# mateog4712/CCJ

Hardware: AMD Instinct MI355X
Metric: sec/sequence + DP-cells/s at n=200 (Turner04), 1/2/4/8 GPU vs CPU ref (higher is better)
Workload: dtype int32

## Files before the change

### ccj_amd/__init__.py

```python
from __future__ import annotations

import ctypes
import os
from typing import Optional

__all__ = [
    "W_final", "ccj", "load_params", "load_par", "ParFileError", "param_path", "CCJError", "BacktrackExit", "lib", "MAT4", "MAT2",
    "num_cells", "comm_unique_id", "shard_blocks", "level_layout", "level_schedule", "LevelSchedule",
    "DEFAULT_SPLIT_TARGET", "LocalGroup", "W_final_pf", "PF_MAT4", "PF_MAT2", "layout_extents", "fold_many",
    "SampleExit", "pf_exp_hashes", "load_pfraw", "LockstepBatch", "batch_level_plan", "BatchLevelPlan", "plan_lockstep",
    "pf_many", "PfLockstepBatch", "pf_level_plan", "PF_PLAN_KERNELS", "pf_setup_host_hashes", "PF_SETUP_TABLES", "RangeError", "RANGE_LEVEL", "RANGE_ILOOP", "RANGE_PARTIAL", "RANGE_TAB", "RANGE_CF", "RANGE_EXIT_CODE",
]

_HERE = os.path.dirname(os.path.abspath(__file__))
_VARIANT = os.environ.get("CCJ_LIB_VARIANT", "")
_LIB_PATH = os.path.join(_HERE, "lib", f"libccj_hip_{_VARIANT}.so" if _VARIANT else "libccj_hip.so")
PARAM_DIR = os.path.join(_HERE, "params")

MAT4 = ["PK", "PL", "PR", "PM", "PO", "PfromL", "PfromR", "PfromM", "PfromMprime", "PfromO",
        "PLmloop00", "PLmloop01", "PLmloop10", "PRmloop00", "PRmloop01", "PRmloop10",
        "PMmloop00", "PMmloop01", "PMmloop10", "POmloop00", "POmloop01", "POmloop10"]
MAT2 = ["P", "WBP", "WPP", "V", "Vtype", "WM", "WMv", "WMp"]
HASH_NAMES = MAT4 + MAT2 + ["W"]
PF_MAT4 = ["PK", "PL", "PR", "PM", "PO", "PfromL", "PfromR", "PfromM", "PfromO",
           "PLmloop00", "PLmloop01", "PLmloop10", "PRmloop00", "PRmloop01", "PRmloop10",
           "PMmloop00", "PMmloop01", "PMmloop10", "POmloop00", "POmloop01", "POmloop10"]
PF_MAT2 = ["V", "VM", "WM", "WMv", "WMp", "WBP", "WPP", "P"]
CCJ_E_PF_SAMPLE = 8
CCJ_E_PF_RANGE = 10

CCJ_OK, CCJ_E_ARG, CCJ_E_OOM, CCJ_E_HIP, CCJ_E_PARAMS, CCJ_E_BACKTRACK, CCJ_E_STATE, CCJ_E_INTER_EXIT = range(8)
CCJ_E_COMM = 9
CCJ_E_PARFILE = 8
CCJ_E_RANGE = 11
RANGE_LEVEL, RANGE_ILOOP, RANGE_PARTIAL, RANGE_TAB, RANGE_CF = 1, 2, 4, 8, 16
RANGE_SITES = {"LEVEL": RANGE_LEVEL, "ILOOP": RANGE_ILOOP, "PARTIAL": RANGE_PARTIAL, "TAB": RANGE_TAB, "CF": RANGE_CF}
RANGE_EXIT_CODE = 3

PARAM_SETS = {
    "Turner04": "Turner04.ccjp", "rna_Turner04": "Turner04.ccjp",
    "DirksPierce09": "DirksPierce09.ccjp", "rna_DirksPierce09": "DirksPierce09.ccjp",
    "DirksPierce03": "DirksPierce03.ccjp", "rna_DirksPierce03": "DirksPierce03.ccjp",
    "CaoChen06": "CaoChen06.ccjp", "rna_CaoChen06": "CaoChen06.ccjp",
    "CaoChen09": "CaoChen09.ccjp", "rna_CaoChen09": "CaoChen09.ccjp",
# ... 171 lines not shown
        L.ccj_pf_reset.restype = ip
        L.ccj_pf_capacity.argtypes = [vp]
        L.ccj_pf_capacity.restype = ip
        L.ccj_pf_n.argtypes = [vp]
        L.ccj_pf_n.restype = ip
        L.ccj_pf_keytab_info.argtypes = [vp, dp, ctypes.POINTER(ctypes.c_ulonglong)]
        L.ccj_pf_keytab_info.restype = ip
        L.ccj_pf_setup_hashes.argtypes = [vp, u64p, ip]
        L.ccj_pf_setup_hashes.restype = ip
        L.ccj_pf_setup_host_hashes.argtypes = [ctypes.POINTER(_Problem), cp, u64p, u64p]
        L.ccj_pf_setup_host_hashes.restype = ip
    if hasattr(L, "ccj_pf_batch_create"):
        L.ccj_pf_batch_create.argtypes = [ctypes.POINTER(_Problem), cp, ip, ip, ip, ctypes.POINTER(vp)]
        L.ccj_pf_batch_create.restype = ip
        L.ccj_pf_batch_bind.argtypes = [vp, ctypes.POINTER(cp), ip]
        L.ccj_pf_batch_bind.restype = ip
        for fn in ("ccj_pf_batch_fill", "ccj_pf_batch_members", "ccj_pf_batch_count", "ccj_pf_batch_launches"):
            getattr(L, fn).argtypes = [vp]
            getattr(L, fn).restype = ip
        L.ccj_pf_batch_result.argtypes = [vp, ip, dp]
        L.ccj_pf_batch_result.restype = ip
        L.ccj_pf_batch_member.argtypes = [vp, ip]
        L.ccj_pf_batch_member.restype = vp
        L.ccj_pf_batch_fill_ms.argtypes = [vp]
        L.ccj_pf_batch_fill_ms.restype = ctypes.c_double
        L.ccj_pf_batch_item_counts.argtypes = [vp, ip, ctypes.POINTER(ip)]
        L.ccj_pf_batch_item_counts.restype = ip
        L.ccj_pf_batch_last_error.argtypes = [vp]
        L.ccj_pf_batch_last_error.restype = cp
        L.ccj_pf_batch_destroy.argtypes = [vp]
        L.ccj_pf_batch_destroy.restype = None
        L.ccj_pf_level_plan_items.argtypes = [ctypes.POINTER(ip), ctypes.POINTER(ip), ip, ip, ctypes.POINTER(ip)]
        L.ccj_pf_level_plan_items.restype = ip
    L.ccj_pf_fill.argtypes = [vp, dp]
    L.ccj_pf_fill.restype = ip
    L.ccj_pf_W.argtypes = [vp, dp]
    L.ccj_pf_W.restype = ip
    L.ccj_pf_get2.argtypes = [vp, ip, dp]
    L.ccj_pf_get2.restype = ip
    L.ccj_pf_get4.argtypes = [vp, ip, ip, ip, ip, ip, ctypes.POINTER(ip)]
    L.ccj_pf_get4.restype = ip
    L.ccj_pf_hashes.argtypes = [vp, u64p, u64p]
    L.ccj_pf_hashes.restype = ip
    L.ccj_pf_exp_hashes.argtypes = [vp, u64p, ip]
    L.ccj_pf_exp_hashes.restype = ip
    L.ccj_pf_exp_hashes_params.argtypes = [cp, cp, vp, u64p, ip]
    L.ccj_pf_exp_hashes_params.restype = ip
    L.ccj_pf_exp_names.argtypes = []
    L.ccj_pf_exp_names.restype = cp
    L.ccj_pf_srand.argtypes = [vp, ctypes.c_uint]
    L.ccj_pf_srand.restype = ip
    L.ccj_pf_sample.argtypes = [vp, ip, cp, ctypes.POINTER(ip)]
    L.ccj_pf_sample.restype = ip
    L.ccj_pf_last_message.argtypes = [vp]
    L.ccj_pf_last_message.restype = cp
    L.ccj_pf_timing.argtypes = [vp, ctypes.POINTER(ctypes.c_float)]
    L.ccj_pf_timing.restype = ip
    L.ccj_pf_set_timing.argtypes = [vp, ip]
    L.ccj_pf_set_timing.restype = ip
    L.ccj_pf_kernel_ms.argtypes = [vp, ctypes.POINTER(ctypes.c_double)]
    L.ccj_pf_kernel_ms.restype = ip
    L.ccj_pf_work_model.argtypes = [vp, ctypes.POINTER(ctypes.c_double)]
    L.ccj_pf_work_model.restype = ip
    _lib = L
    return L


def num_cells(n: int) -> int:
    if n < 3:
        return 0
    m = n + 1
    return m * (m - 1) * (m - 2) * (m - 3) // 24


def param_path(name_or_path: str) -> str:
    if os.path.exists(name_or_path) and name_or_path.endswith(".ccjp"):
        return name_or_path
    base = os.path.basename(name_or_path)
    for suf in (".par", ".ccjp"):
        if base.endswith(suf):
            base = base[: -len(suf)]
    if base in PARAM_SETS:
        return os.path.join(PARAM_DIR, PARAM_SETS[base])
    raise CCJError(CCJ_E_ARG, f"unknown parameter set {name_or_path!r}")


class ParFileError(CCJError):

    def __init__(self, log: str):
        super().__init__(CCJ_E_PARFILE, log)
        self.log = log


def load_par(path: str, base: bytes | None = None, text: bool = False):
    if base is None:
        base = _read_blob(os.path.join(PARAM_DIR, "default.ccjp"))
    L = lib()
    out = ctypes.create_string_buffer(len(base))
    cap = 1 << 22
    log = ctypes.create_string_buffer(cap)
    fn = L.ccj_params_load_par_string if text else L.ccj_params_load_par
    rc = fn(path.encode(), bytes(base), out, log, cap)
    msg = log.value.decode(errors="replace")
    if rc == CCJ_E_PARFILE:
        raise ParFileError(msg)
# ... 66 lines not shown

    def reset(self, seq: str) -> None:
        if len(seq) != self.n:
            raise CCJError(CCJ_E_ARG, f"reset: length {len(seq)} differs from n={self.n}")
        self._check(lib().ccj_reset(self._h, seq.encode()))
        self.seq = seq
        self._seq_buf = ctypes.create_string_buffer(seq.encode())
        self.structure = None
        self.energy = None
        self.stdout_msgs = ""

    def rebind(self, seq: str) -> None:
        self._check(lib().ccj_rebind(self._h, seq.encode()))
        self.seq = seq
        self.n = len(seq)
        self._seq_buf = ctypes.create_string_buffer(seq.encode())
        self.structure = None
        self.energy = None
        self.stdout_msgs = ""

    @property
    def capacity(self) -> int:
        return lib().ccj_capacity(self._h)

    def _check(self, rc: int):
        if rc == CCJ_E_RANGE:
            raise RangeError(rc, lib().ccj_last_error(self._h).decode(), self.range_flags())
        if rc != CCJ_OK:
            raise CCJError(rc, lib().ccj_last_error(self._h).decode())

    def range_flags(self) -> int:
        return lib().ccj_range_flags(self._h)

    def fill(self):
        self._check(lib().ccj_fill(self._h))

    def fill_device(self):
        self._check(lib().ccj_fill_device(self._h))

    def sync_host(self):
        self._check(lib().ccj_sync_host(self._h))

    def result(self):
        L = lib()
        buf = ctypes.create_string_buffer(self.n + 1)
        msgs = ctypes.create_string_buffer(1 << 16)
        e = ctypes.c_double()
        rc = L.ccj_result(self._h, buf, ctypes.byref(e), msgs, 1 << 16)
        self.stdout_msgs = msgs.value.decode()
        if rc == CCJ_E_BACKTRACK or rc == CCJ_E_INTER_EXIT:
            err = L.ccj_last_error(self._h).decode()
            exit_code = 0 if rc == CCJ_E_INTER_EXIT else (134 if "Assertion" in err else 1)
            raise BacktrackExit(rc, err, exit_code, self.stdout_msgs)
        self._check(rc)
        self.structure = buf.value.decode()
        self.energy = e.value
        return self.energy

    def ccj(self) -> float:
        self.fill()
        return self.result()

    def fill_async(self, after: Optional["W_final"] = None) -> None:
        if after is None:
            self._check(lib().ccj_fill_async(self._h))
        else:
# ... 692 lines not shown
```

### ccj_amd/csrc/ccj_host.cc

```cpp
#include <hip/hip_runtime.h>
#include <rccl/rccl.h>

#include <algorithm>
#include <atomic>
#include <chrono>
#include <condition_variable>
#include <mutex>
#include <cmath>
#include <cstdarg>
#include <cstdio>
#include <cstdlib>
#include <cstring>
#include <list>
#include <memory>
#include <stack>
#include <string>
#include <thread>
#include <vector>

#include "ccj.h"
#include "ccj_energy.h"
#include "ccj_engine.h"
#include "ccj_backtrack.h"
#include "ccj_traceback.h"
#include "ccj_items.h"

using namespace ccj;

namespace {

const int BP_PAIR[8][8] = {{0, 0, 0, 0, 0, 0, 0, 0}, {0, 0, 0, 0, 5, 0, 0, 5}, {0, 0, 0, 1, 0, 0, 0, 0},
                           {0, 0, 2, 0, 3, 0, 0, 0}, {0, 6, 0, 4, 0, 0, 0, 6}, {0, 0, 0, 0, 0, 0, 2, 0},
                           {0, 0, 0, 0, 0, 1, 0, 0}, {0, 6, 0, 0, 5, 0, 0, 0}};

template <class T>
struct DevBuf {
    T *p = nullptr;
    size_t count = 0;
};

}

struct ccj_group {
    int world = 1;
    std::vector<ccj_ctx *> members;
    std::mutex mu;
    std::condition_variable cv;
    int arrived = 0;
    long gen = 0;
    bool broken = false;
    int busy = 0;
    int range_acc[2] = {0, 0};
    bool barrier() {
        std::unique_lock<std::mutex> lk(mu);
        if (broken) return false;
        const long g = gen;
        if (++arrived == world) {
            arrived = 0;
// ... 1890 lines not shown

extern "C" int ccj_work_model(const ccj_ctx *c, double *out) {
    if (!c || !out) return CCJ_E_ARG;
    double w[5];
    const int rc = work_model(c->n, c->S.data(), c->pair, w);
    for (int x = 0; x < 4; ++x) out[x] = w[x];
    return rc;
}

extern "C" int ccj_work_split(const ccj_ctx *c, double *out2) {
    if (!c || !out2) return CCJ_E_ARG;
    double w[5];
    const int rc = work_model(c->n, c->S.data(), c->pair, w);
    out2[0] = 2.0 * w[4];
    out2[1] = w[0] - out2[0];
    return rc;
}

extern "C" int ccj_work_model_seq(const char *seq, int noGU, double *out) {
    if (!seq || !out) return CCJ_E_ARG;
    const int n = (int)strlen(seq);
    int pairt[8][8];
    for (int x = 0; x < 8; ++x)
        for (int y = 0; y < 8; ++y) pairt[x][y] = BP_PAIR[x][y];
    if (noGU) pairt[3][4] = pairt[4][3] = 0;
    std::vector<short> S(n + 2, 0);
    for (int i = 1; i <= n; ++i) S[i] = (short)encode_base(seq[i - 1]);
    double w[5];
    const int rc = work_model(n, S.data(), pairt, w);
    for (int x = 0; x < 4; ++x) out[x] = w[x];
    return rc;
}

extern "C" int ccj_host_timing(const ccj_ctx *c, double *out3) {
    if (!c || !out3) return CCJ_E_ARG;
    out3[0] = c->sync_ms;
    out3[1] = c->w_ms;
    out3[2] = c->bt_ms;
    return CCJ_OK;
}

extern "C" int ccj_level_times(const ccj_ctx *c, double *level_ms, double *diag_ms, int cap) {
    if (!c) return CCJ_E_ARG;
    for (int t = 0; t < cap && t < (int)c->lev_ms_v.size(); ++t) {
        if (level_ms) level_ms[t] = c->lev_ms_v[t];
        if (diag_ms) diag_ms[t] = c->diag_ms_v[t];
    }
    return CCJ_OK;
}

extern "C" int ccj_iloop_times(const ccj_ctx *c, double *iloop_ms, int cap) {
    if (!c || !iloop_ms) return CCJ_E_ARG;
    for (int t = 0; t < cap && t < (int)c->il_ms_v.size(); ++t) iloop_ms[t] = c->il_ms_v[t];
    return CCJ_OK;
}

extern "C" int ccj_exchange_times(const ccj_ctx *c, double *edge_ms, double *bulk_ms, int cap) {
    if (!c || (!edge_ms && !bulk_ms)) return CCJ_E_ARG;
    for (int t = 0; t < cap && t < (int)c->xch_ms_v.size(); ++t) {
        if (edge_ms) edge_ms[t] = c->xch_ms_v[t];
        if (bulk_ms) bulk_ms[t] = c->xbulk_ms_v[t];
    }
    return CCJ_OK;
}

extern "C" double ccj_iloop_ms(const ccj_ctx *c) { return c ? c->il_ms : 0.0; }
// ... 499 lines not shown
```

### ccj_amd/csrc/ccj_kernels.hip

```cpp
#include <hip/hip_runtime.h>
#include <stdlib.h>
#include "ccj_engine.h"
#include "ccj_energy.h"
#include "ccj_items.h"

using namespace ccj;

#ifdef CCJ_WG_TIMELINE
constexpr int TL_CAP = 1 << 15, TL_KINDS = 8;
__device__ int g_tl_level = -1;
__device__ ulonglong4 g_tl[TL_KINDS][TL_CAP];
struct TLStamp {
    int slot;
    unsigned long long t0;
    unsigned meta = 0xffffffffu;
    template <class K>
    __device__ __forceinline__ explicit TLStamp(K kind_of) {
        const int kind = kind_of(g_tl_level);
        const int wpb = (int)(blockDim.x >> 6);
        const int s = (int)blockIdx.x * wpb + (int)(threadIdx.x >> 6);
        slot = (g_tl_level >= 0 && kind >= 0 && s < TL_CAP && (threadIdx.x & 63) == 0) ? kind * TL_CAP + s : -1;
        t0 = __builtin_amdgcn_s_memrealtime();
    }
    __device__ __forceinline__ ~TLStamp() {
        if (slot < 0) return;
        const unsigned long long t1 = __builtin_amdgcn_s_memrealtime();
        const unsigned hw = __builtin_amdgcn_s_getreg((31 << 11) | 4);
        (&g_tl[0][0])[slot] = make_ulonglong4(t0, t1, meta, hw | (unsigned long long)(blockIdx.x % 8) << 32);
    }
};
#define TL_STAMP(expr_) TLStamp tl_stamp_([&](int L_) -> int { return (expr_); })
#define TL_META(v_) (tl_stamp_.meta = (unsigned)(v_))
#else
#define TL_STAMP(expr_)
#define TL_META(v_)
#endif

// ... 109 lines not shown
            if (e != INF) e += E_MLstem(P, tt, -1, -1) + P->MLclosing;
            break;
    }
    return e;
}

}

__device__ __forceinline__ void init2d_body(const DevTables &T, int total) {
    for (int x = blockIdx.x * blockDim.x + threadIdx.x; x < total; x += gridDim.x * blockDim.x) {
        T.V[x] = 10000;
        T.Vt[x] = 'N';
        T.WM[x] = T.WMv[x] = T.WMp[x] = INF + 1;
        T.P[x] = T.WBP[x] = T.WPP[x] = INF + 1;
        T.Pk[x] = ~0ull;
        T.WB[x] = 0;
        T.WP[x] = 0;
        T.WBW[x] = make_int2(INF + 1, 0);
#pragma unroll
        for (int f = 0; f < 6; ++f) T.tab[f * T.tabN + x] = (int16_t)INTERN_INF;
#pragma unroll
        for (int f = 0; f < NCF; ++f) T.cf[f * T.tabN + x] = INF;
    }
}
__global__ void k_init2d(DevTables T, int total) { init2d_body(T, total); }
__global__ void k_init2d_many(const DevTables *__restrict__ tabs) {
    const DevTables &T = tabs[blockIdx.y];
    init2d_body(T, (T.n + 1) * T.rs);
}

__device__ __forceinline__ int e_intP(const DevTables &T, int u1, int u2, int p, int q) {
    const int d = p + u1 + 1, dp = q - u2 - 1;
    if (dp - d < 1) return INTERN_INF;
    const int t1 = T.pair[T.S[p] * 8 + T.S[q]];
    const int t2 = T.pair[T.S[d] * 8 + T.S[dp]];
    if (t1 <= 0 || t2 <= 0) return INTERN_INF;
    const int e = E_IntLoop(T.prm, T.lx, u1, u2, t1, T.rtype[t2], T.S1[p + 1], T.S1[q - 1], T.S1[d - 1], T.S1[dp + 1]);
    const int v = (int)rint(T.e_intP * (double)e);
    if (v < -32768 || v >= INTERN_INF) atomicOr(T.err, 1);
    return v;
}

__device__ __forceinline__ void precompute_ie_body(const DevTables &T) {
    const int n = T.n, rs = T.rs;
    const int w = blockIdx.y;
    for (int p = 1 + blockIdx.x * blockDim.x + threadIdx.x; p + w <= n; p += gridDim.x * blockDim.x)
        T.ie[(size_t)w * rs + p] = (int16_t)e_intP(T, 0, 0, p, p + w);
}
__global__ void k_precompute_ie(DevTables T) { precompute_ie_body(T); }
__global__ void k_precompute_ie_many(const DevTables *__restrict__ tabs) { precompute_ie_body(tabs[blockIdx.z]); }

__device__ __forceinline__ void diag2d_tables(const DevTables &T, int sigma, int item) {
    const int n = T.n, rs = T.rs, w = sigma;
    const int p = 1 + item, q = p + w;
    if (q > n) return;
    const int lane = threadIdx.x & 63;
    const int cp = T.pen.cp;
    const int16_t *F00 = T.tab, *F10 = T.tab + 2 * T.tabN, *G00 = T.tab + 3 * T.tabN;
    Mloop2dAcc L = mloop2d_begin(T.pen.bp), R = L;
    for (int s = 1 + lane; s <= w; s += 64) {
#ifdef CCJ_DEBUG_BOUNDS
        if (p + s > n || q - s + 1 < 1 || w - s < 0) atomicOr(T.err, 512);
#endif
        const int head = T.WBW[(s - 1) * rs + p].x, tail = T.WBW[(s - 1) * rs + q - s + 1].x;
        const int o = (w - s) * rs + p;
        mloop2d_step(L, true, s, w, cp, head, tail, F00[o + s], F00[o], F10[o]);
        mloop2d_step(R, false, s, w, cp, head, tail, G00[o + s], G00[o], 0);
    }
    L.m00 = wave_min(L.m00); L.m01 = wave_min(L.m01); L.m10 = wave_min(L.m10);
    R.m00 = wave_min(R.m00); R.m01 = wave_min(R.m01); R.m10 = wave_min(R.m10);
    if (lane != 0) return;
    if (w >= 1) {
// ... 414 lines not shown
                for (int s = 0; s < PP_S; ++s) {
                    const int code = (live && s < ns && hh[u] <= o0 + s) ? 1023 - hh[u] : PP_OFF;
                    bv[s] = imin(bv[s], ((va[u][s] + vb[u]) << 10) + code);
                }
            }
        }
#pragma unroll
        for (int s = 0; s < PP_S; ++s) {
            const int sg = lev + 3 + o0 + s;
            const int i = l - sg;
            if (s < ns && l <= n && i >= 1 && bv[s] < (PP_OFF >> 1)) {
                const unsigned h2 = 1023u - (unsigned)(bv[s] & 1023);
                const unsigned jo = (unsigned)(o0 + s) - h2, dd = jo + 1u + (unsigned)a2, ko = dd + 1u + h2;
                const unsigned key = (jo * (unsigned)sg + dd) * (unsigned)sg + ko;
                atomicMin(T.Pk + sg * rs + i, ((unsigned long long)((unsigned)(bv[s] >> 10) + 0x80000000u) << 32) | key);
            }
        }
    }
}
constexpr int PPUSH_HS = 32;
template <int PP_S, int PP_U>
__global__ __launch_bounds__(256) void k_ppush(DevTables T, int lev, int ngrp, int npairs, int hs_len, int blocksA, int G,
                                               int rank, int nout) {
    ppush_body<PP_S, PP_U>(T, lev, ngrp, npairs, hs_len, blocksA, G, rank, nout);
}
template <int PP_S, int PP_U>
__global__ __launch_bounds__(256) void k_ppush_many(const DevTables *__restrict__ tabs, const LevelArgs *__restrict__ args,
                                                    int lev) {
    const LevelArgs &A = args[blockIdx.y];
    if ((int)blockIdx.x >= 2 * A.pp_blocksA) return;
    ppush_body<PP_S, PP_U>(tabs[blockIdx.y], lev, A.pp_ngrp, A.pp_npairs, PPUSH_HS, A.pp_blocksA, 1, 0, A.pp_nout);
}

__device__ __forceinline__ void build_il_body(const DevTables &T, int kind) {
    __shared__ int16_t es[IE_U][IE_U + 1];
    __shared__ uint32_t vb[IE_U];
    const int n = T.n, rs = T.rs;
    const int p = blockIdx.x + 1, w = blockIdx.y;
    const int q = p + w;
    if (q > n) return;
    if (T.pt[(size_t)w * rs + p] <= 0) return;
    const int lane = threadIdx.x;
    const size_t pidx = (size_t)w * rs + p;
    uint32_t *seg = (kind ? T.ilmseg : T.ilseg) + pidx * IL_SEG;
    uint2 *ent = (kind ? T.ilm : T.il) + pidx * IL_CAP;
    if (lane < IE_U) {
        const int u1 = lane;
        uint32_t bits = 0;
#pragma unroll
        for (int u2 = 0; u2 < IE_U; ++u2) {
            bool valid = false;
            int e = 0;
            if (kind == 0) {
                const int d = p + 1 + u1, dp = q - 1 - u2;
                if (u1 <= imin(w, MAXLOOP) - 2 && u2 <= imin(w - u1 - 6, MAXLOOP - 2) && T.pt[(dp - d) * rs + d] > 0) {
                    valid = true;
                    e = e_intP(T, u1, u2, p, q);
                }
            } else {
                const int d = p - 1 - u1, dp = q + 1 + u2;
                if (d >= 1 && dp <= n && T.pt[(dp - d) * rs + d] > 0) {
                    valid = true;
                    e = e_intP(T, u1, u2, d, dp);
                }
            }
            es[u1][u2] = (int16_t)e;
            bits |= (valid ? 1u : 0u) << u2;
        }
        vb[u1] = bits;
    }
    __syncthreads();
    int cnt = 0;
    for (int dt = 0; dt < IL_SEG; ++dt) {
        if (lane == 0) seg[dt] = (uint32_t)cnt;
        const int u1 = lane, u2 = dt - 2 - lane;
        const bool valid = dt >= 2 && u1 < IE_U && u2 >= 0 && u2 < IE_U && ((vb[u1] >> u2) & 1u);
        const unsigned long long mask = __ballot(valid);
        if (valid)
            ent[cnt + __popcll(mask & ((1ull << lane) - 1))] =
                make_uint2(((uint32_t)dt << 21) | ((uint32_t)u1 << 16) | (uint32_t)(uint16_t)es[u1][u2], (uint32_t)(2 * u1 * dt));
        cnt += __popcll(mask);
    }
    if (lane < IL_B) ent[cnt + lane] = make_uint2((63u << 21) | (uint32_t)INTERN_INF, 0u);
}
__global__ __launch_bounds__(64) void k_build_il(DevTables T) { build_il_body(T, (int)blockIdx.z); }
__global__ __launch_bounds__(64) void k_build_il_many(const DevTables *__restrict__ tabs) {
    build_il_body(tabs[blockIdx.z >> 1], (int)(blockIdx.z & 1));
}

struct DevPT {
    const DevTables *T;
    __device__ int operator()(int i, int j) const { return ptype(*T, i, j); }
};

__global__ __launch_bounds__(256) void k_items(DevTables T, int G, int rank, int simulate,
                                               long long *counts, const long long *__restrict__ offs, uint32_t *items,
                                               int pass) {
    __shared__ int wsum[4];
    __shared__ long long tot;
    const int bs = blockIdx.x, b = bs / KI_SPLIT, sp = bs - b * KI_SPLIT, t = b / G, r = b - t * G;
    const int tid = threadIdx.x, lane = tid & 63, w = tid >> 6;
    const bool mine = simulate || r == rank;
    if (!mine || t < 4 || t >= T.nlev) {
        if (pass == 0 && tid == 0) counts[bs] = 0;
        return;
    }
    const ItemRows R = item_rows(T.n, t, G, r);
    const DevPT pt{&T};
    int lo, hi;
    ki_split_rows(R.nPL + R.nPR + R.nPM, sp, lo, hi);
    long long base = pass ? offs[bs] : 0;
    for (int c0 = lo; c0 < hi; c0 += 256) {
        const int x = c0 + tid;
        uint32_t it0 = 0;
        const int cnt = x < hi ? item_row(pt, T.n, t, R, x, G, r, it0, IL_CW) : 0;
        int inc = cnt;
#pragma unroll
        for (int o = 1; o < 64; o <<= 1) {
            const int y = __shfl_up(inc, o, 64);
            if (lane >= o) inc += y;
// ... 1088 lines not shown
}

static bool ppush_geom(int n, int lev, int G, int rank, int &ngrp, int &npairs, int &nout, int &blocksA) {
    ngrp = npairs = nout = blocksA = 0;
    const int nmax = imin(lev, n - 4 - lev) + 1;
    if (nmax <= 0) return false;
    ngrp = (n - lev - 3 + 63) / 64;
    constexpr int S = PPUSH_S, hs_len = PPUSH_HS;
    const int nch = (nmax + S - 1) / S;
    for (int c = 0; c < nch; ++c) npairs += (imin((c + 1) * S, nmax) + hs_len - 1) / hs_len;
    nout = rank <= lev ? (lev - rank) / G + 1 : 0;
    if (nout <= 0) return false;
    blocksA = (npairs * ngrp * nout + 3) / 4;
    return true;
}

extern "C" int ccjk_ppush(const DevTables *T, int lev, int G, int rank, void *stream) {
#ifdef CCJ_ABLATE_PTERM
    return 0;
#endif
    constexpr int S = PPUSH_S, hs_len = PPUSH_HS;
    int ngrp, npairs, nout, blocksA;
    if (!ppush_geom(T->n, lev, G, rank, ngrp, npairs, nout, blocksA)) return 0;
    static const int steps = getenv("CCJ_PP_STEPS") ? atoi(getenv("CCJ_PP_STEPS")) : 4;
    if (steps >= 4)
        hipLaunchKernelGGL((k_ppush<S, 4>), dim3((unsigned)(2 * blocksA)), dim3(256), 0, (hipStream_t)stream, *T, lev, ngrp,
                           npairs, hs_len, blocksA, G, rank, nout);
    else
        hipLaunchKernelGGL((k_ppush<S, 2>), dim3((unsigned)(2 * blocksA)), dim3(256), 0, (hipStream_t)stream, *T, lev, ngrp,
                           npairs, hs_len, blocksA, G, rank, nout);
    return (int)hipGetLastError();
}

extern "C" int ccjk_build_il(const DevTables *T, void *stream) {
    const int n = T->n;
    if (n < 1) return 0;
    hipLaunchKernelGGL(k_build_il, dim3(n, n + 1, 2), dim3(64), 0, (hipStream_t)stream, *T);
    return (int)hipGetLastError();
}

extern "C" int ccjk_iloop(const DevTables *T, int t, long long first_item, int nitems, int G, int rank, void *stream) {
#ifdef CCJ_ABLATE_ILOOP
    return 0;
#endif
    if (nitems <= 0) return 0;
    hipLaunchKernelGGL(k_iloop, dim3((unsigned)((nitems + IL_WPB - 1) / IL_WPB)), dim3(64 * IL_WPB), 0, (hipStream_t)stream, *T, t, first_item,
                       nitems, G, rank);
    return (int)hipGetLastError();
}

__global__ __launch_bounds__(256) void k_pack(DevTables T, int t, int G, int r, int part, int nmax, int16_t *send) {
    const int n = T.n, m = n - t - 2, Mt = (m * (m + 1)) >> 1;
    const long long gc = (long long)blockIdx.x * blockDim.x + threadIdx.x;
    const int k = (int)(gc / Mt);
    if (k >= xch_pcount(t, G, r, part)) return;
    const int c = (int)(gc - (long long)k * Mt);
    const LvlDev Lt = T.ld[t];
    const int16_t *src = T.d4 + Lt.lb + (long long)shard_a(xch_own(k, part), G, r) * Mt + c;
#pragma unroll 2
    for (int x = 0; x < NMAT4; ++x) {
        const bool own = carrier(x) == IN_D4 || carrier(x) == IN_REC;
        send[xch_pos(x, k, c, nmax, Mt)] = own ? src[(long long)mslot(x) * Lt.C] : (int16_t)INTERN_INF;
    }
}

__global__ __launch_bounds__(256) void k_unpack(DevTables T, int t, int G, int r, int part, int nmax, const int16_t *recv,
                                                size_t rstride) {
    const int n = T.n, m = n - t - 2, Mt = (m * (m + 1)) >> 1;
    const long long gc = (long long)blockIdx.x * blockDim.x + threadIdx.x;
    const int a = (int)(gc / Mt);
// ... 259 lines not shown
    for (int k = 0; k < count; ++k) {
        const int m = n[k] - t - 2;
        if (m > 0) total += (long)(t + 1) * ((m * (m + 1) / 2 + 63) / 64);
    }
    BatchLevelPlan P{0, 0, 0, 0};
    if (total <= 0 || t < 0) {
        for (int k = 0; k < count; ++k) {
            if (blocks) blocks[k] = 0;
            if (wpa) wpa[k] = 0;
        }
        return P;
    }
    P.split = sched_split_of(total, split_target);
    P.threads = P.split <= 4 ? 256 : 64 * P.split;
    const int cpb = P.threads / 64 / P.split;
    P.lds = P.split > 1 ? cpb * (P.split - 1) * SPLIT_RED * 64 * (int)sizeof(int) : 0;
    for (int k = 0; k < count; ++k) {
        const int m = n[k] - t - 2;
        const int w = m > 0 ? (m * (m + 1) / 2 + 63) / 64 : 0;
        const long b = ((long)(m > 0 ? t + 1 : 0) * w + cpb - 1) / cpb;
        if (blocks) blocks[k] = (int)b;
        if (wpa) wpa[k] = w;
        P.gridx = b > P.gridx ? (int)b : P.gridx;
    }
    return P;
}

extern "C" int ccjk_pre_many(const DevTables *tabs, int count, int nmax, void *stream) {
    if (count <= 0 || nmax < 1) return 0;
    const hipStream_t s = (hipStream_t)stream;
    const int total = (nmax + 1) * (nmax + 2);
    hipLaunchKernelGGL(k_init2d_many, dim3((total + 255) / 256, count), dim3(256), 0, s, tabs);
    hipLaunchKernelGGL(k_precompute_ie_many, dim3((nmax + 255) / 256, nmax + 1, count), dim3(256), 0, s, tabs);
    hipLaunchKernelGGL(k_build_il_many, dim3(nmax, nmax + 1, 2 * count), dim3(64), 0, s, tabs);
    return (int)hipGetLastError();
}

extern "C" int ccjk_iloop_many(const DevTables *tabs, const LevelArgs *row, const LevelArgs *hrow, int count, int t, void *stream) {
    int gx = 0;
    for (int k = 0; k < count; ++k) gx = imax(gx, (hrow[k].il_nitems + IL_WPB - 1) / IL_WPB);
    if (gx <= 0) return 0;
    hipLaunchKernelGGL(k_iloop_many, dim3(gx, count), dim3(64 * IL_WPB), 0, (hipStream_t)stream, tabs, row, t);
    return (int)hipGetLastError();
}

extern "C" int ccjk_diag2d_many(const DevTables *tabs, const LevelArgs *row, const LevelArgs *hrow, int count, int sigma,
                                void *stream) {
    int gx = 0;
    for (int k = 0; k < count; ++k) gx = imax(gx, hrow[k].dg_blocks);
    if (gx <= 0) return 0;
    hipLaunchKernelGGL(k_diag2d_many, dim3(gx, count), dim3(256), 0, (hipStream_t)stream, tabs, row, sigma);
    return (int)hipGetLastError();
}

extern "C" int ccjk_level4d_many(const DevTables *tabs, const LevelArgs *row, const int *n, int count, int t, int split_target,
                                 void *stream) {
    const BatchLevelPlan P = ccjk_batch_level_plan(n, count, t, split_target, nullptr, nullptr);
    if (P.gridx <= 0) return 0;
    hipLaunchKernelGGL(k_level4d_many, dim3((unsigned)P.gridx, count), dim3(P.threads), (size_t)P.lds, (hipStream_t)stream, tabs,
                       row, t, P.split);
    return (int)hipGetLastError();
}

extern "C" int ccjk_ppush_many(const DevTables *tabs, const LevelArgs *row, const LevelArgs *hrow, int count, int lev,
                               void *stream) {
#ifdef CCJ_ABLATE_PTERM
    return 0;
// ... 23 lines not shown
```

### include/ccj.h

```cpp
#ifndef CCJ_H
#define CCJ_H

#include <stdint.h>
#include "ccj_params.h"

#ifdef __cplusplus
extern "C" {
#endif

#define CCJ_OK           0
#define CCJ_E_ARG        1
#define CCJ_E_OOM        2
#define CCJ_E_HIP        3
#define CCJ_E_PARAMS     4
#define CCJ_E_BACKTRACK  5
#define CCJ_E_STATE      6
#define CCJ_E_INTER_EXIT 7
#define CCJ_E_COMM       9
#define CCJ_E_RANGE     11

#define CCJ_RANGE_LEVEL   1
#define CCJ_RANGE_ILOOP   2
#define CCJ_RANGE_PARTIAL 4
#define CCJ_RANGE_TAB     8
// ... 83 lines not shown
int  ccj_iloop_times(const ccj_ctx *ctx, double *iloop_ms, int cap);
int  ccj_ppush_times(const ccj_ctx *ctx, double *ppush_ms, int cap);
int  ccj_set_timing(ccj_ctx *ctx, int mode);

#define CCJ_COMM_ID_BYTES 128
int  ccj_comm_unique_id(char *id_out);
int  ccj_comm_init(ccj_ctx *ctx, const char *id);
int  ccj_shard_blocks(int n, int t, int world, int rank, int *a_out, int cap);
int  ccj_level_layout(int n, int t, int world, long long *C, int *M);
int  ccj_level_schedule(int n, int t, int world, int rank, int split_target, int share, int *out5);
int  ccj_ctx_level_schedule(const ccj_ctx *ctx, int t, int rank, int *out7);
int  ccj_exchange_layout(int n, int t, int world, int part, long long *out3);
long long ccj_exchange_index(int n, int t, int world, int rank, int part, int which, long long *out, long long cap);
typedef struct ccj_group ccj_group;
int  ccj_group_create(int world, ccj_group **out);
void ccj_group_destroy(ccj_group *g);
int  ccj_comm_init_local(ccj_ctx *ctx, ccj_group *g);

int  ccj_work_model(const ccj_ctx *ctx, double *out4);
int  ccj_work_split(const ccj_ctx *ctx, double *out2);
int  ccj_work_model_seq(const char *seq, int noGU, double *out4);

int  ccj_n(const ccj_ctx *ctx);
const char *ccj_last_error(const ccj_ctx *ctx);
int  ccj_range_flags(const ccj_ctx *ctx);
void ccj_destroy(ccj_ctx *ctx);

uint64_t ccj_num_cells(int n);

long long ccj_pmpo2d_closed(int n, const int *wbp, int bp, int cp, int16_t *out, long long cells);
int  ccj_pmpo2d_low(int n, const int *wbp, int bp, int cp, int *out6);
int  ccj_pmpo2d_low_brute(int n, const int *wbp, int bp, int cp, int valid_only, int *out6);

#ifdef __cplusplus
}
#endif

#endif
```

Baseline: 2.339 billion.

## Prune dominated interior-loop window entries when building IL tables

When the interior-loop (IL) candidate tables are built, each (u1,u2) entry is now checked against a shorter or stacked decomposition, and any entry that one of those dominates is removed before compaction. This shrinks the per-pair IL entry lists that the fill kernels scan. The pruning is on by default and can be turned off with CCJ_IL_PRUNE=0. It adds shared-memory work and syncs to the build kernel and relies on the dominance argument being exact, which a new host reference and count APIs are there to check.

After: 2.788 billion, median of 6. 19.2% higher.

```diff
diff --git a/ccj_amd/__init__.py b/ccj_amd/__init__.py
--- a/ccj_amd/__init__.py
+++ b/ccj_amd/__init__.py
@@ -10,6 +10,7 @@
     "DEFAULT_SPLIT_TARGET", "LocalGroup", "W_final_pf", "PF_MAT4", "PF_MAT2", "layout_extents", "fold_many",
     "SampleExit", "pf_exp_hashes", "load_pfraw", "LockstepBatch", "batch_level_plan", "BatchLevelPlan", "plan_lockstep",
     "pf_many", "PfLockstepBatch", "pf_level_plan", "PF_PLAN_KERNELS", "pf_setup_host_hashes", "PF_SETUP_TABLES", "RangeError", "RANGE_LEVEL", "RANGE_ILOOP", "RANGE_PARTIAL", "RANGE_TAB", "RANGE_CF", "RANGE_EXIT_CODE",
+    "il_prune_host", "IL_U",
 ]
 
 _HERE = os.path.dirname(os.path.abspath(__file__))
@@ -247,6 +248,11 @@
         L.ccj_pf_batch_destroy.restype = None
         L.ccj_pf_level_plan_items.argtypes = [ctypes.POINTER(ip), ctypes.POINTER(ip), ip, ip, ctypes.POINTER(ip)]
         L.ccj_pf_level_plan_items.restype = ip
+    if hasattr(L, "ccj_il_counts"):
+        L.ccj_il_counts.argtypes = [vp, ctypes.POINTER(ctypes.c_longlong)]
+        L.ccj_il_counts.restype = ip
+        L.ccj_il_prune_host.argtypes = [ctypes.POINTER(_Problem), ctypes.POINTER(ctypes.c_longlong)] + [vp] * 6
+        L.ccj_il_prune_host.restype = ip
     L.ccj_pf_fill.argtypes = [vp, dp]
     L.ccj_pf_fill.restype = ip
     L.ccj_pf_W.argtypes = [vp, dp]
@@ -286,6 +292,37 @@
         return 0
     m = n + 1
     return m * (m - 1) * (m - 2) * (m - 3) // 24
+
+
+IL_U = 29
+
+
+def il_prune_host(seq: str, params: str | bytes = "Turner04", dangle: int = 2, noGU: bool = False, pen=None,
+                  windows: bool = True):
+    import numpy as np
+    blob = params if isinstance(params, (bytes, bytearray)) else load_params(params)
+    blob_buf = ctypes.create_string_buffer(bytes(blob), len(blob))
+    seq_buf = ctypes.create_string_buffer(seq.encode())
+    pk = None
+    if pen is not None:
+        pk = _Penalties(*[int(v) for v in pen[:12]], float(pen[12]), float(pen[13]))
+    prob = _Problem(ctypes.cast(seq_buf, ctypes.c_char_p), dangle, 1 if noGU else 0, ctypes.cast(blob_buf, ctypes.c_void_p),
+                    ctypes.cast(ctypes.pointer(pk), ctypes.c_void_p) if pk is not None else None)
+    n = len(seq)
+    counts = (ctypes.c_longlong * 4)()
+    out = {}
+    ptrs = [None] * 6
+    if windows:
+        shape = (n + 1, n + 2, IL_U, IL_U)
+        for x, (name, dt, sh) in enumerate([("e_il", np.int16, shape), ("e_ilm", np.int16, shape), ("st_il", np.uint8, shape),
+                                            ("st_ilm", np.uint8, shape), ("est", np.int16, shape[:2]), ("ie", np.int16, shape[:2])]):
+            out[name] = np.zeros(sh, dtype=dt)
+            ptrs[x] = out[name].ctypes.data_as(ctypes.c_void_p)
+    rc = lib().ccj_il_prune_host(ctypes.byref(prob), counts, *ptrs)
+    if rc != CCJ_OK:
+        raise CCJError(rc, "ccj_il_prune_host")
+    out["counts"] = tuple(counts)
+    return out
 
 
 def param_path(name_or_path: str) -> str:
@@ -418,6 +455,11 @@
     def range_flags(self) -> int:
         return lib().ccj_range_flags(self._h)
 
+    def il_counts(self):
+        out = (ctypes.c_longlong * 4)()
+        self._check(lib().ccj_il_counts(self._h, out))
+        return tuple(out)
+
     def fill(self):
         self._check(lib().ccj_fill(self._h))
 
diff --git a/ccj_amd/csrc/ccj_host.cc b/ccj_amd/csrc/ccj_host.cc
--- a/ccj_amd/csrc/ccj_host.cc
+++ b/ccj_amd/csrc/ccj_host.cc
@@ -24,6 +24,7 @@
 #include "ccj_backtrack.h"
 #include "ccj_traceback.h"
 #include "ccj_items.h"
+#include "ccj_ilprune.h"
 
 using namespace ccj;
 
@@ -1980,6 +1981,106 @@
     return rc;
 }
 
+extern "C" int ccj_il_counts(ccj_ctx *c, long long *out4) {
+    if (!c || !out4) return CCJ_E_ARG;
+    if (!c->filled) return set_err(c, CCJ_E_STATE, "ccj_il_counts before a fill");
+    HIPCHK(c, hipSetDevice(c->device));
+    const size_t plane = (size_t)(c->n + 1) * c->rs;
+    std::vector<uint32_t> seg(plane * IL_SEG);
+    for (int kind = 0; kind < 2; ++kind) {
+        HIPCHK(c, hipMemcpy(seg.data(), kind ? c->d_ilmseg : c->d_ilseg, seg.size() * sizeof(uint32_t), hipMemcpyDeviceToHost));
+        long long kept = 0, full = 0;
+        for (int w = 0; w < c->n; ++w)
+            for (int p = 1; p + w <= c->n; ++p) {
+                const size_t x = (size_t)w * c->rs + p;
+                if (c->hpt_h[x] <= 0) continue;
+                kept += seg[x * IL_SEG + IL_SEG - 1];
+                full += seg[x * IL_SEG];
+            }
+        out4[2 * kind] = kept;
+        out4[2 * kind + 1] = full;
+    }
+    return CCJ_OK;
+}
+
+extern "C" int ccj_il_prune_host(const ccj_problem *prob, long long *counts4, int16_t *e_il, int16_t *e_ilm, uint8_t *st_il,
+                                 uint8_t *st_ilm, int16_t *est_out, int16_t *ie_out) {
+    if (!prob || !prob->seq || !prob->params) return CCJ_E_ARG;
+    const int n = (int)strlen(prob->seq), rs = n + 2;
+    if (n < 1 || prob->params->magic != CCJ_PARAMS_MAGIC || prob->params->size_bytes != sizeof(ccj_energy_params)) return CCJ_E_ARG;
+    ccj_pk_penalties pk = CCJ_PK_PENALTIES_DEFAULT;
+    if (prob->pen) pk = *prob->pen;
+    int8_t pair[64], rtype[8] = {0, 2, 1, 4, 3, 6, 5, 7};
+    for (int x = 0; x < 8; ++x)
+        for (int y = 0; y < 8; ++y) pair[x * 8 + y] = (int8_t)BP_PAIR[x][y];
+    if (prob->noGU) pair[3 * 8 + 4] = pair[4 * 8 + 3] = 0;
+    for (int x = 0; x < 8; ++x)
+        for (int y = 0; y < 8; ++y) rtype[pair[x * 8 + y]] = pair[y * 8 + x];
+    std::vector<short> S(n + 2, 0), S1(n + 2, 0);
+    for (int i = 1; i <= n; ++i) S[i] = S1[i] = (short)encode_base(prob->seq[i - 1]);
+    S[n + 1] = S[1], S[0] = (short)n, S1[n + 1] = S1[1], S1[0] = S1[n];
+    std::vector<int> lx((size_t)2 * n + 64, 0);
+    for (size_t x = 31; x < lx.size(); ++x) lx[x] = (int)(prob->params->lxc * log((double)x / 30.));
+    const size_t plane = (size_t)(n + 1) * rs;
+    std::vector<int8_t> pt(plane, 0);
+    std::vector<int16_t> est(plane, (int16_t)INTERN_INF), ie(plane, (int16_t)INTERN_INF);
+    const IlHostTables T{n, rs, S.data(), S1.data(), pt.data(), pair, rtype, prob->params, lx.data(), pk.e_intP, est.data(), ie.data()};
+    bool bad = false;
+    for (int w = 0; w < n; ++w)
+        for (int p = 1; p + w <= n; ++p) {
+            const int q = p + w;
+            const size_t x = (size_t)w * rs + p;
+            pt[x] = pair[S[p] * 8 + S[q]];
+            if (q - p >= 2 && p + 1 != q - 1) {
+                const int t2 = pair[S[p + 1] * 8 + S[q - 1]];
+                const long v = lrint(pk.e_stP * E_IntLoop(prob->params, lx.data(), 0, 0, pt[x], rtype[t2], S1[p + 1], S1[q - 1], S1[p], S1[q]));
+                if (v < -32768 || (pt[x] > 0 && t2 > 0 && v >= INTERN_INF)) bad = true;
+                est[x] = (int16_t)(v >= INTERN_INF ? INTERN_INF : v);
+            }
+            const int v = il_eint_raw(T, 0, 0, p, q);
+            if (v != INTERN_INF && !il_e_in_range(v)) bad = true;
+            ie[x] = (int16_t)v;
+        }
+    if (bad) return CCJ_E_PARAMS;
+    long long cnt[4] = {0, 0, 0, 0};
+    int es[IE_U][IE_U];
+    bool in[IE_U][IE_U];
+    for (int kind = 0; kind < 2; ++kind) {
+        int16_t *eo = kind ? e_ilm : e_il;
+        uint8_t *so = kind ? st_ilm : st_il;
+        if (eo) memset(eo, 0, plane * IE_U * IE_U * sizeof(int16_t));
+        if (so) memset(so, 0, plane * IE_U * IE_U);
+        for (int w = 0; w < n; ++w)
+            for (int p = 1; p + w <= n; ++p) {
+                const size_t x = (size_t)w * rs + p;
+                if (pt[x] <= 0) continue;
+                const int q = p + w;
+                for (int u1 = 0; u1 < IE_U; ++u1)
+                    for (int u2 = 0; u2 < IE_U; ++u2) {
+                        es[u1][u2] = 0;
+                        in[u1][u2] = il_window(T, kind, p, q, u1, u2, es[u1][u2]);
+                        if (in[u1][u2] && !il_e_in_range(es[u1][u2])) return CCJ_E_PARAMS;
+                    }
+                for (int u1 = 0; u1 < IE_U; ++u1)
+                    for (int u2 = 0; u2 < IE_U; ++u2) {
+                        if (!in[u1][u2]) continue;
+                        const int dom = (u1 && u2) ? il_dominated(T, kind, p, q, u1, u2, es[u1][u2], in[0][0], es[0][0],
+                                                                  in[u1 - 1][u2 - 1], es[u1 - 1][u2 - 1])
+                                                   : 0;
+                        cnt[2 * kind] += dom == 0;
+                        cnt[2 * kind + 1] += 1;
+                        const size_t o = (x * IE_U + u1) * IE_U + u2;
+                        if (eo) eo[o] = (int16_t)es[u1][u2];
+                        if (so) so[o] = (uint8_t)(1 | 2 * dom);
+                    }
+            }
+    }
+    if (counts4) memcpy(counts4, cnt, sizeof cnt);
+    if (est_out) memcpy(est_out, est.data(), plane * sizeof(int16_t));
+    if (ie_out) memcpy(ie_out, ie.data(), plane * sizeof(int16_t));
+    return CCJ_OK;
+}
+
 extern "C" int ccj_host_timing(const ccj_ctx *c, double *out3) {
     if (!c || !out3) return CCJ_E_ARG;
     out3[0] = c->sync_ms;
diff --git a/ccj_amd/csrc/ccj_ilprune.h b/ccj_amd/csrc/ccj_ilprune.h
--- /dev/null
+++ b/ccj_amd/csrc/ccj_ilprune.h
@@ -0,0 +1,77 @@
+#pragma once
+#include <cmath>
+#include <cstdint>
+#include "ccj_energy.h"
+
+namespace ccj {
+
+constexpr int IL_NEAR = 1, IL_FAR = 2;
+
+template <class TB>
+CCJ_HD int il_eint_raw(const TB &T, int u1, int u2, int p, int q) {
+    const int d = p + u1 + 1, dp = q - u2 - 1;
+    if (dp - d < 1) return INTERN_INF;
+    const int t1 = T.pair[T.S[p] * 8 + T.S[q]];
+    const int t2 = T.pair[T.S[d] * 8 + T.S[dp]];
+    if (t1 <= 0 || t2 <= 0) return INTERN_INF;
+    const int e = E_IntLoop(T.prm, T.lx, u1, u2, t1, T.rtype[t2], T.S1[p + 1], T.S1[q - 1], T.S1[d - 1], T.S1[dp + 1]);
+    return (int)rint(T.e_intP * (double)e);
+}
+CCJ_HD bool il_e_in_range(int v) { return v >= -32768 && v < INTERN_INF; }
+
+template <class TB>
+CCJ_HD bool il_window(const TB &T, int kind, int p, int q, int u1, int u2, int &e) {
+    const int w = q - p, rs = T.rs;
+    if (kind == 0) {
+        const int d = p + 1 + u1, dp = q - 1 - u2;
+        if (!(u1 <= imin(w, MAXLOOP) - 2 && u2 <= imin(w - u1 - 6, MAXLOOP - 2) && T.pt[(dp - d) * rs + d] > 0)) return false;
+        e = il_eint_raw(T, u1, u2, p, q);
+    } else {
+        const int d = p - 1 - u1, dp = q + 1 + u2;
+        if (!(d >= 1 && dp <= T.n && T.pt[(dp - d) * rs + d] > 0)) return false;
+        e = il_eint_raw(T, u1, u2, d, dp);
+    }
+    return true;
+}
+
+template <class TB>
+CCJ_HD int il_stack00(const TB &T, int x, int y) {
+    const int o = (y - x) * T.rs + x;
+    return imin((int)T.est[o], (int)T.ie[o]);
+}
+
+template <class TB>
+CCJ_HD int il_dominated(const TB &T, int kind, int p, int q, int u1, int u2, int E, bool v00, int e00, bool vprev, int eprev) {
+    if (u1 < 1 || u2 < 1 || !il_e_in_range(E)) return 0;
+    const int d = kind ? p - 1 - u1 : p + 1 + u1, dp = kind ? q + 1 + u2 : q - 1 - u2;
+    const int sN = kind ? il_stack00(T, p - 1, q + 1) : il_stack00(T, p, q);
+    const int sF = kind ? il_stack00(T, d, dp) : il_stack00(T, d - 1, dp + 1);
+    const bool one = u1 == 1 && u2 == 1;
+    int bits = 0;
+    if (vprev && il_e_in_range(eprev)) {
+        const int E1 = one ? sN : eprev;
+        if (E1 + sF <= E) bits |= IL_FAR;
+    }
+    if (v00 && il_e_in_range(e00)) {
+        int E2 = sF;
+        if (!one) {
+            if (bits) return bits;
+            E2 = kind ? il_eint_raw(T, u1 - 1, u2 - 1, d, dp) : il_eint_raw(T, u1 - 1, u2 - 1, p + 1, q - 1);
+            if (!il_e_in_range(E2)) return bits;
+        }
+        if (sN + E2 <= E) bits |= IL_NEAR;
+    }
+    return bits;
+}
+
+struct IlHostTables {
+    int n, rs;
+    const short *S, *S1;
+    const int8_t *pt, *pair, *rtype;
+    const ccj_energy_params *prm;
+    const int *lx;
+    double e_intP;
+    const int16_t *est, *ie;
+};
+
+}
diff --git a/ccj_amd/csrc/ccj_kernels.hip b/ccj_amd/csrc/ccj_kernels.hip
--- a/ccj_amd/csrc/ccj_kernels.hip
+++ b/ccj_amd/csrc/ccj_kernels.hip
@@ -3,6 +3,7 @@
 #include "ccj_engine.h"
 #include "ccj_energy.h"
 #include "ccj_items.h"
+#include "ccj_ilprune.h"
 
 using namespace ccj;
 
@@ -178,12 +179,9 @@
 __device__ __forceinline__ int e_intP(const DevTables &T, int u1, int u2, int p, int q) {
     const int d = p + u1 + 1, dp = q - u2 - 1;
     if (dp - d < 1) return INTERN_INF;
-    const int t1 = T.pair[T.S[p] * 8 + T.S[q]];
-    const int t2 = T.pair[T.S[d] * 8 + T.S[dp]];
-    if (t1 <= 0 || t2 <= 0) return INTERN_INF;
-    const int e = E_IntLoop(T.prm, T.lx, u1, u2, t1, T.rtype[t2], T.S1[p + 1], T.S1[q - 1], T.S1[d - 1], T.S1[dp + 1]);
-    const int v = (int)rint(T.e_intP * (double)e);
-    if (v < -32768 || v >= INTERN_INF) atomicOr(T.err, 1);
+    if (T.pair[T.S[p] * 8 + T.S[q]] <= 0 || T.pair[T.S[d] * 8 + T.S[dp]] <= 0) return INTERN_INF;
+    const int v = il_eint_raw(T, u1, u2, p, q);
+    if (!il_e_in_range(v)) atomicOr(T.err, 1);
     return v;
 }
 
@@ -664,7 +662,7 @@
     ppush_body<PP_S, PP_U>(tabs[blockIdx.y], lev, A.pp_ngrp, A.pp_npairs, PPUSH_HS, A.pp_blocksA, 1, 0, A.pp_nout);
 }
 
-__device__ __forceinline__ void build_il_body(const DevTables &T, int kind) {
+__device__ __forceinline__ void build_il_body(const DevTables &T, int kind, int prune) {
     __shared__ int16_t es[IE_U][IE_U + 1];
     __shared__ uint32_t vb[IE_U];
     const int n = T.n, rs = T.rs;
@@ -702,9 +700,28 @@
         vb[u1] = bits;
     }
     __syncthreads();
+    int full = lane < IE_U ? __popc(vb[lane]) : 0;
+#pragma unroll
+    for (int o = 32; o > 0; o >>= 1) full += __shfl_xor(full, o, 64);
+    if (prune) {
+        uint32_t dom = 0;
+        if (lane >= 1 && lane < IE_U) {
+            const int u1 = lane;
+            const uint32_t mine = vb[u1], prev = vb[u1 - 1];
+            const bool v00 = vb[0] & 1u;
+            const int e00 = es[0][0];
+            for (int u2 = 1; u2 < IE_U; ++u2)
+                if (((mine >> u2) & 1u) &&
+                    il_dominated(T, kind, p, q, u1, u2, es[u1][u2], v00, e00, (prev >> (u2 - 1)) & 1u, es[u1 - 1][u2 - 1]))
+                    dom |= 1u << u2;
+        }
+        __syncthreads();
+        if (lane < IE_U) vb[lane] &= ~dom;
+        __syncthreads();
+    }
     int cnt = 0;
     for (int dt = 0; dt < IL_SEG; ++dt) {
-        if (lane == 0) seg[dt] = (uint32_t)cnt;
+        if (lane == 0) seg[dt] = dt ? (uint32_t)cnt : (uint32_t)full;
         const int u1 = lane, u2 = dt - 2 - lane;
         const bool valid = dt >= 2 && u1 < IE_U && u2 >= 0 && u2 < IE_U && ((vb[u1] >> u2) & 1u);
         const unsigned long long mask = __ballot(valid);
@@ -715,9 +732,9 @@
     }
     if (lane < IL_B) ent[cnt + lane] = make_uint2((63u << 21) | (uint32_t)INTERN_INF, 0u);
 }
-__global__ __launch_bounds__(64) void k_build_il(DevTables T) { build_il_body(T, (int)blockIdx.z); }
-__global__ __launch_bounds__(64) void k_build_il_many(const DevTables *__restrict__ tabs) {
-    build_il_body(tabs[blockIdx.z >> 1], (int)(blockIdx.z & 1));
+__global__ __launch_bounds__(64) void k_build_il(DevTables T, int prune) { build_il_body(T, (int)blockIdx.z, prune); }
+__global__ __launch_bounds__(64) void k_build_il_many(const DevTables *__restrict__ tabs, int prune) {
+    build_il_body(tabs[blockIdx.z >> 1], (int)(blockIdx.z & 1), prune);
 }
 
 struct DevPT {
@@ -1872,10 +1889,15 @@
     return (int)hipGetLastError();
 }
 
+static int il_prune_on() {
+    const char *e = getenv("CCJ_IL_PRUNE");
+    return !(e && atoi(e) == 0);
+}
+
 extern "C" int ccjk_build_il(const DevTables *T, void *stream) {
     const int n = T->n;
     if (n < 1) return 0;
-    hipLaunchKernelGGL(k_build_il, dim3(n, n + 1, 2), dim3(64), 0, (hipStream_t)stream, *T);
+    hipLaunchKernelGGL(k_build_il, dim3(n, n + 1, 2), dim3(64), 0, (hipStream_t)stream, *T, il_prune_on());
     return (int)hipGetLastError();
 }
 
@@ -2201,7 +2223,7 @@
     const int total = (nmax + 1) * (nmax + 2);
     hipLaunchKernelGGL(k_init2d_many, dim3((total + 255) / 256, count), dim3(256), 0, s, tabs);
     hipLaunchKernelGGL(k_precompute_ie_many, dim3((nmax + 255) / 256, nmax + 1, count), dim3(256), 0, s, tabs);
-    hipLaunchKernelGGL(k_build_il_many, dim3(nmax, nmax + 1, 2 * count), dim3(64), 0, s, tabs);
+    hipLaunchKernelGGL(k_build_il_many, dim3(nmax, nmax + 1, 2 * count), dim3(64), 0, s, tabs, il_prune_on());
     return (int)hipGetLastError();
 }
 
diff --git a/include/ccj.h b/include/ccj.h
--- a/include/ccj.h
+++ b/include/ccj.h
@@ -139,6 +139,10 @@
 int  ccj_pmpo2d_low(int n, const int *wbp, int bp, int cp, int *out6);
 int  ccj_pmpo2d_low_brute(int n, const int *wbp, int bp, int cp, int valid_only, int *out6);
 
+int  ccj_il_counts(ccj_ctx *ctx, long long *out4);
+int  ccj_il_prune_host(const ccj_problem *prob, long long *counts4, int16_t *e_il, int16_t *e_ilm, uint8_t *st_il,
+                       uint8_t *st_ilm, int16_t *est, int16_t *ie);
+
 #ifdef __cplusplus
 }
 #endif
```
